# BaptisteHudyma/RGB-D-SLAM

Measured on AMD Instinct MI355X. Metric: depth frames/s primitive extraction (640x480), higher is better.
Workload: dtype f64; 1 GPU; 640x480 synthetic planar-room depth stream, plane extraction only (BASELINE.json configs[1]); stream_frames=4096, unique_frames_per_gpu=4096, scene=room, sub_batches=0, frames_rendered_on=device (torch)

## Files before the change

rgb-d-slam_amd/csrc/cape_cell_acc.h:

```cpp
#pragma once
#include <hip/hip_runtime.h>

#include "cape_device.h"
#include "cape_internal.h"

namespace cape {


#ifndef CAPE_A_GROUP
#define CAPE_A_GROUP 2
#endif
#ifndef CAPE_A_WAVES
#define CAPE_A_WAVES 4
#endif

constexpr int kThreadsA = 320;
constexpr int kBandThreads = 160;
[[maybe_unused]] constexpr int kPartStride = 11;

struct PxAcc
{
    double S[9];
    uint32_t n;
    uint32_t zminBits1, zmaxBits;
};

__device__ __forceinline__ float acc_px(float zr, double a, double b, PxAcc& A)
{
    const bool valid = zr > 0.0f;
    const float z = valid ? zr : 0.0f;
    A.n += valid ? 1u : 0u;
    const double zd = (double)z;
    const float x = (float)(zd * a);
    const float y = (float)(zd * b);
    A.S[0] += (double)x;
    A.S[1] += (double)y;
    A.S[2] += zd;
    A.S[3] += (double)(x * x);
    A.S[4] += (double)(y * y);
    A.S[5] += (double)(z * z);
    A.S[6] += (double)(x * y);
    A.S[7] += (double)(y * z);
    A.S[8] += (double)(x * z);
    return z;
}

__device__ __forceinline__ uint32_t acc_px_fast(float z, double a, double b, PxAcc& A)
{
    const uint32_t bits = __float_as_uint(z);
    A.n += min(bits, 1u);
    const double zd = (double)z;
    const float x = (float)(zd * a);
    const float y = (float)(zd * b);
    A.S[0] += (double)x;
    A.S[1] += (double)y;
    A.S[2] += zd;
    A.S[3] += (double)(x * x);
    A.S[4] += (double)(y * y);
    A.S[5] += (double)(z * z);
    A.S[6] += (double)(x * y);
    A.S[7] += (double)(y * z);
    A.S[8] += (double)(x * z);
    return bits;
}

__device__ __forceinline__ void acc_f4(const float4& v, double a0, double a1, double a2, double a3, double b, PxAcc& A)
{
    const uint32_t bx = acc_px_fast(v.x, a0, b, A);
    const uint32_t by = acc_px_fast(v.y, a1, b, A);
    const uint32_t bz = acc_px_fast(v.z, a2, b, A);
    const uint32_t bw = acc_px_fast(v.w, a3, b, A);
    A.zmaxBits = max(max(A.zmaxBits, bx), max(by, max(bz, bw)));
    A.zminBits1 = min(min(A.zminBits1, bx - 1u), min(by - 1u, min(bz - 1u, bw - 1u)));
}

__device__ __forceinline__ bool is_continuous(float pixelDepth, float& last)
{
    if (pixelDepth > 0)
    {
        if ((double)fabsf(pixelDepth - last) <= 4.0 * depth_quantization((double)pixelDepth))
        {
            last = pixelDepth;
            return true;
        }
        return false;
    }
    return true;
}

__device__ __forceinline__ bool is_continuous_flat(float pixelDepth, float& last)
{
    const bool positive = pixelDepth > 0;
    const bool close = (double)fabsf(pixelDepth - last) <= 4.0 * depth_quantization((double)pixelDepth);
    last = (positive & close) ? pixelDepth : last;
    return !positive | close;
}

}
```

rgb-d-slam_amd/csrc/cape_cell_moments.hip:

```cpp
#include <hip/hip_runtime.h>

#include <type_traits>

#include "cape_cell_acc.h"

namespace cape {

template <bool U16> __global__ __launch_bounds__(kThreadsA, CAPE_A_WAVES) void cape_cell_moments_kernel(StageAParams p)
{
    __shared__ double s_part[kThreadsA * kPartStride];
    __shared__ float s_row[64 * kCell];
    __shared__ float s_col[64 * kCell];
    __shared__ float s_corner[64 * 2];
    __shared__ float s_trash[kThreadsA + kCell];

    const int t = threadIdx.x;
    const int frame = blockIdx.x / p.pairsPerFrame;
    const int pair = blockIdx.x - frame * p.pairsPerFrame;
    const size_t frameOff = (size_t)frame * p.W * p.H;

    const int bsel = t / kBandThreads;
    const int q = t - bsel * kBandThreads;
    const int band = pair * 2 + bsel;
    const int cellRow = band / p.segsPerRow;
    const int seg = band - cellRow * p.segsPerRow;
    const int col0 = seg * 640 + q * 4;
    const bool active = (band < p.bandsPerFrame) && (col0 < p.W);
    const int cseg = q / 5;
    const int j = q - cseg * 5;
    const int lcell = bsel * 32 + cseg;

    PxAcc A;
#pragma unroll
    for (int k = 0; k < 9; ++k)
        A.S[k] = 0.0;
    A.n = 0;
    A.zminBits1 = 0xFFFFFFFFu;
    A.zmaxBits = 0u;
    if (active)
    {
        const double a0 = p.acol[col0], a1 = p.acol[col0 + 1], a2 = p.acol[col0 + 2], a3 = p.acol[col0 + 3];
        const uint32_t pixOff32 = (uint32_t)(cellRow * kCell) * (uint32_t)p.W + (uint32_t)col0;
        const float* frameBase = p.depth + frameOff;
        const uint16_t* frameBase16 = p.depth_u16 + frameOff;
        const float scale16 = p.u16_scale;
        const double* brow = p.brow + cellRow * kCell;
        const size_t W = (size_t)p.W;

        constexpr int kGroup = CAPE_A_GROUP, kGroups = kCell / kGroup;
        static_assert(kCell % kGroup == 0 && kGroups % 2 == 0, "the ping-pong loop consumes two groups per trip");
        using Raw = typename std::conditional<U16, ushort4, float4>::type;
        Raw bufA[kGroup], bufB[kGroup];
        auto load_group = [&](Raw (&buf)[kGroup], int g) {
#pragma unroll
            for (int i = 0; i < kGroup; ++i)
            {
                const size_t rowOff = (size_t)(kGroup * g + i) * W;
                if constexpr (U16)
                {
                    typedef unsigned short u16x4 __attribute__((ext_vector_type(4)));
                    const u16x4 v = __builtin_nontemporal_load(reinterpret_cast<const u16x4*>((frameBase16 + rowOff) + pixOff32));
                    buf[i] = make_ushort4(v.x, v.y, v.z, v.w);
                }
                else
                {
                    typedef float f32x4 __attribute__((ext_vector_type(4)));
                    const f32x4 v = __builtin_nontemporal_load(reinterpret_cast<const f32x4*>((frameBase + rowOff) + pixOff32));
                    buf[i] = make_float4(v.x, v.y, v.z, v.w);
                }
            }
        };
        auto to_f4 = [&](const Raw& rw) {
            if constexpr (U16)
            {
                return make_float4((float)rw.x * scale16, (float)rw.y * scale16, (float)rw.z * scale16, (float)rw.w * scale16);
            }
            else
            {
                return rw;
            }
        };
        float* const colp = (j == 2) ? &s_col[lcell * kCell] : &s_trash[t];
        auto sum_group = [&](const Raw (&rawbuf)[kGroup], int g, auto where) {
            constexpr int kWhere = decltype(where)::value;
            float4 buf[kGroup];
#pragma unroll
            for (int i = 0; i < kGroup; ++i)
                buf[i] = to_f4(rawbuf[i]);
#pragma unroll
            for (int i = 0; i < kGroup; ++i)
            {
                const int r = kGroup * g + i;
                acc_f4(buf[i], a0, a1, a2, a3, brow[r], A);
                colp[r] = buf[i].z;
                if (kWhere == 1 && r == kCell / 2)
                    *reinterpret_cast<float4*>(&s_row[lcell * kCell + 4 * j]) = buf[i];
                if (kWhere == 0 && i == 0 && g == 0 && j == 0)
                    s_corner[lcell * 2] = buf[i].x;
                if (kWhere == 2 && r == kCell - 1 && j == 4)
                    s_corner[lcell * 2 + 1] = buf[i].w;
            }
        };
        using First = std::integral_constant<int, 0>;
        using Loop = std::integral_constant<int, 1>;
        using Last = std::integral_constant<int, 2>;
        static_assert(kGroups >= 6 && (kCell / 2) / kGroup >= 2 && (kCell / 2) / kGroup < kGroups - 2, "row 10 belongs to a trip of the loop");
        load_group(bufA, 0);
        load_group(bufB, 1);
        sum_group(bufA, 0, First{});
        load_group(bufA, 2);
        sum_group(bufB, 1, First{});
#pragma unroll 1
        for (int g = 2; g < kGroups - 2; g += 2)
        {
            load_group(bufB, g + 1);
            sum_group(bufA, g, Loop{});
            load_group(bufA, g + 2);
            sum_group(bufB, g + 1, Loop{});
        }
        load_group(bufB, kGroups - 1);
        sum_group(bufA, kGroups - 2, Last{});
        sum_group(bufB, kGroups - 1, Last{});
    }
    {
        double* dst = s_part + t * kPartStride;
#pragma unroll
        for (int k = 0; k < 9; ++k)
            dst[k] = A.S[k];
        dst[9] = (double)A.n;
        reinterpret_cast<uint2*>(dst + 10)[0] = make_uint2(A.zminBits1, A.zmaxBits);
    }
    __syncthreads();

    if (t >= 256)
    {
        const int l = t - 256;
        size_t base[2];
        int lim[2];
#pragma unroll
        for (int cb = 0; cb < 2; ++cb)
        {
            const int bnd = pair * 2 + cb;
            const int cr = bnd / p.segsPerRow;
            const int sg = bnd - cr * p.segsPerRow;
            base[cb] = (size_t)frame * p.cells + cr * p.hCells + sg * 32;
            lim[cb] = bnd < p.bandsPerFrame ? p.hCells - sg * 32 : 0;
        }
#pragma unroll
        for (int k = 0; k < 10; ++k)
        {
            const int e = l + 64 * k;
            const int cell = e / 10;
            const int m = e - cell * 10;
            const int cb = cell >> 5, cs = cell & 31;
            if (cs < (cb ? lim[1] : lim[0]))
            {
                const double* src = s_part + (cb * kBandThreads + cs * 5) * kPartStride + m;
                double acc = src[0];
                acc += src[kPartStride];
                acc += src[2 * kPartStride];
                acc += src[3 * kPartStride];
                acc += src[4 * kPartStride];
                p.cell_sums[((cb ? base[1] : base[0]) + cs) * kSumStride + m] = acc;
            }
        }
        return;
    }

    const int w = t >> 6, l = t & 63;
    const int c64 = w * 16 + (l & 15);
    const bool vertical = (l & 32) != 0;
    const bool second = (l & 16) != 0;
    bool continuous;
    {
        const float* zs = (vertical ? s_col : s_row) + c64 * kCell;
        const float seed = std_maxf(zs[0], zs[1]);
        float last = seed;
#pragma unroll
        for (int i = 1; i <= 9; ++i)
        {
            const float z = zs[i];
            last = (second && z > 0) ? z : last;
        }
        continuous = second || !(seed <= 0);
        const float* zt = zs + (second ? 10 : 1);
        const int steps = second ? (vertical ? 9 : 10) : 9;
#pragma unroll
        for (int k = 0; k < 10; ++k)
        {
            const bool pass = is_continuous_flat(zt[k], last);
            continuous &= pass | (k >= steps);
        }
        continuous &= __shfl_xor((int)continuous, 16) != 0;
        continuous &= __shfl_xor((int)continuous, 32) != 0;
    }
    const int fb = c64 >> 5, fs = c64 & 31;
    const int fband = pair * 2 + fb;
    if ((l >> 4) != 0 || fband >= p.bandsPerFrame)
        return;
    const int fRow = fband / p.segsPerRow;
    const int fSeg = fband - fRow * p.segsPerRow;
    const int fCol = fSeg * 32 + fs;
    if (fCol >= p.hCells)
        return;
    uint32_t zminBits1 = 0xFFFFFFFFu, zmaxBits = 0u;
    uint32_t n = 0;
    {
        const int pbase = fb * kBandThreads + fs * 5;
#pragma unroll
        for (int k = 0; k < 5; ++k)
        {
            const uint2 zr = reinterpret_cast<const uint2*>(s_part + (pbase + k) * kPartStride + 10)[0];
            zminBits1 = min(zminBits1, zr.x);
            zmaxBits = max(zmaxBits, zr.y);
            n += (uint32_t)s_part[(pbase + k) * kPartStride + 9];
        }
    }
    const float zmin = __uint_as_float(zminBits1 + 1u), zmax = __uint_as_float(zmaxBits);
    const float rab = fmaxf(p.ratio_col[fCol], p.ratio_row[fRow]);
    const bool exact_ok = zmaxBits <= 0x7F7FFFFFu && ((n == 0) || (zmax * rab <= 512.0f * zmin));

    const size_t gcell = (size_t)frame * p.cells + fRow * p.hCells + fCol;
    CellAux aux;
    aux.z0 = s_corner[c64 * 2];
    aux.z399 = s_corner[c64 * 2 + 1];
    aux.flags = (n & kCountMask) | (continuous ? kAuxContinuous : 0u) | (exact_ok ? kAuxExact : 0u);
    aux.zc = s_row[c64 * kCell + kCell / 2];
    p.cell_aux[gcell] = aux;
}

hipError_t launch_cell_moments(const StageAParams& p, int nFrames, hipStream_t stream)
{
    const int grid = nFrames * p.pairsPerFrame;
    if (p.depth)
        hipLaunchKernelGGL(cape_cell_moments_kernel<false>, dim3(grid), dim3(kThreadsA), 0, stream, p);
    else
        hipLaunchKernelGGL(cape_cell_moments_kernel<true>, dim3(grid), dim3(kThreadsA), 0, stream, p);
    return hipGetLastError();
}

}
```

Baseline: 2.325 million frames/s.

## Use f32 continuity test with f64 fallback and hoist band indexing to scalars

Replaces the per-pixel f64 depth-continuity check in the scan waves with an f32 polynomial check. The check flags near-threshold cases, and the wave falls back to the exact f64 path only if any lane is unsure. Band row/segment/offset calculations are computed once per block as wave-uniform scalars via readfirstlane, which removes per-thread integer divisions. The reduce wave is restructured so each element index serves both bands. A profiling script that inventories VALU instructions by kernel region is added. The f32 path risks divergence from the f64 results only inside the guarded margin, and the fallback costs a second pass when triggered.

```diff
diff --git a/profiles/a1_inventory.py b/profiles/a1_inventory.py
--- /dev/null
+++ b/profiles/a1_inventory.py
@@ -0,0 +1,101 @@
+#!/usr/bin/env python3
+import argparse
+import os
+import re
+import subprocess
+import sys
+
+sys.path.insert(0, os.path.dirname(os.path.abspath(__file__)))
+from valu_issue import CSRC, RATE_NS, classify
+
+SYMBOLS = (("f32", "_ZN4cape24cape_cell_moments_kernelILb0EEEvNS_12StageAParamsE"),
+           ("u16", "_ZN4cape24cape_cell_moments_kernelILb1EEEvNS_12StageAParamsE"))
+ORDER = ("prologue", "first trips", "loop trip", "last trips", "partial store", "reduce wave", "scan waves", "scan f64 redo", "aux store")
+WEIGHT = {"prologue": 1, "first trips": 1, "loop trip": 3, "last trips": 1, "partial store": 1, "reduce wave": 0.2, "scan waves": 0.8,
+          "scan f64 redo": 0.0, "aux store": 0.8}
+
+
+def find(body, lo, pred):
+    return next(i for i in range(lo, len(body)) if pred(body[i]))
+
+
+def regions(asm, symbol):
+    start = next(i for i, ln in enumerate(asm) if ln.startswith(symbol + ":"))
+    end = find(asm, start, lambda ln: "s_endpgm" in ln)
+    body = asm[start + 1:end + 1]
+    is_depth_load = lambda ln: re.search(r"global_load_dwordx[24] .* nt$", ln.rstrip()) is not None
+    first_load = find(body, 0, is_depth_load)
+    head = find(body, 0, lambda ln: "Loop Header" in ln)
+    label = body[head].split(":")[0]
+    loop_end = find(body, head, lambda ln: re.search(r"s_c?branch\w*\s+" + re.escape(label) + r"\b", ln) is not None)
+    skip = re.search(r"s_cbranch_execz\s+(\S+)", body[find(body, 0, lambda ln: "s_cbranch_execz" in ln)]).group(1)
+    join = find(body, loop_end, lambda ln: ln.startswith(skip + ":"))
+    barrier = find(body, join, lambda ln: "s_barrier" in ln)
+    out = {"prologue": body[:first_load], "first trips": body[first_load:head], "loop trip": body[head:loop_end + 1],
+           "last trips": body[loop_end + 1:join], "partial store": body[join:barrier + 1]}
+    br = find(body, barrier, lambda ln: re.search(r"s_cbranch_\w+\s+\.LBB", ln) is not None)
+    target = re.search(r"(\.LBB\w+)", body[br]).group(1)
+    split = find(body, br, lambda ln: ln.startswith(target + ":"))
+    arms = [body[barrier + 1:split], body[split:]]
+    reduce_arm = next(a for a in arms if any("global_store_dwordx2" in ln for ln in a))
+    scan_arm = next(a for a in arms if a is not reduce_arm)
+    out["reduce wave"] = reduce_arm
+    last_perm = max(i for i, ln in enumerate(scan_arm) if "ds_bpermute_b32" in ln)
+    scan, redo = scan_arm[:last_perm + 1], []
+    for i, ln in enumerate(scan):
+        m = re.search(r"s_cbranch_vccz\s+(\.LBB\w+)", ln)
+        if m:
+            j = find(scan, i, lambda x: x.startswith(m.group(1) + ":"))
+            if any(re.search(r"v_cmp_\w+_f64", x) for x in scan[i:j]):
+                scan, redo = scan[:i + 1] + scan[j:], scan[i + 1:j]
+                break
+    out["scan waves"], out["scan f64 redo"], out["aux store"] = scan, redo, scan_arm[last_perm + 1:]
+    return out
+
+
+def count(lines):
+    c = {"f64": 0, "double_rate": 0, "other": 0}
+    for ln in lines:
+        m = re.match(r"\s+(v_\w+)", ln)
+        if m:
+            c[classify(m.group(1))] += 1
+    return c
+
+
+def inventory(asm):
+    res = {}
+    for variant, symbol in SYMBOLS:
+        res[variant] = {name: count(lines) for name, lines in regions(asm, symbol).items()}
+    return res
+
+
+def priced(c):
+    return sum(c[k] * RATE_NS[k] for k in RATE_NS)
+
+
+def main():
+    ap = argparse.ArgumentParser()
+    ap.add_argument("--asm", default="")
+    args = ap.parse_args()
+    path = args.asm
+    if not path:
+        path = "/tmp/cape_cell_moments.inventory.s"
+        flags = "-O3 -std=c++17 -fPIC --offload-arch=gfx950 -ffp-contract=off -fno-fast-math -fno-slp-vectorize".split()
+        subprocess.check_call(["/opt/rocm/bin/hipcc"] + flags + ["-S", "--cuda-device-only", "-o", path, os.path.join(CSRC, "cape_cell_moments.hip")],
+                              stderr=subprocess.DEVNULL)
+    inv = inventory(open(path).read().splitlines())
+    for variant, regs in inv.items():
+        print(f"{variant}   VALU instructions as listed                      f64-rate  double-rate  other   total   runs/wave   issue ns/wave")
+        tot_n = tot_ns = 0.0
+        for name in ORDER:
+            c = regs[name]
+            n = c["f64"] + c["double_rate"] + c["other"]
+            ns = priced(c) * WEIGHT[name]
+            tot_n += n * WEIGHT[name]
+            tot_ns += ns
+            print(f"  {name:<48} {c['f64']:8d} {c['double_rate']:12d} {c['other']:6d} {n:7d} {WEIGHT[name]:11.1f} {ns:15.1f}")
+        print(f"  {'per wave, weighted':<48} {'':8} {'':12} {'':6} {tot_n:7.0f} {'':11} {tot_ns:15.1f}")
+
+
+if __name__ == "__main__":
+    main()
diff --git a/rgb-d-slam_amd/csrc/cape_cell_acc.h b/rgb-d-slam_amd/csrc/cape_cell_acc.h
--- a/rgb-d-slam_amd/csrc/cape_cell_acc.h
+++ b/rgb-d-slam_amd/csrc/cape_cell_acc.h
@@ -96,4 +96,19 @@
     return !positive | close;
 }
 
+__device__ __forceinline__ bool is_continuous_flat_f32(float pixelDepth, float& last, bool& unsure)
+{
+    constexpr float c2 = (float)(4.0 * (2.73 * ((1.0 / 1000.0) * (1.0 / 1000.0))));
+    constexpr float c1 = (float)(4.0 * (0.74 / 1000.0));
+    constexpr float c0 = (float)(4.0 * -0.53);
+    const bool positive = pixelDepth > 0;
+    const float r = fmaxf(fmaf(fmaf(c2, pixelDepth, c1), pixelDepth, c0), 2.0f);
+    const float t = fabsf(pixelDepth - last) - r;
+    const bool notSure = !(fabsf(t) > r * 0x1p-16f);
+    const bool close = t <= 0;
+    unsure |= positive & notSure;
+    last = (positive & close) ? pixelDepth : last;
+    return !positive | close;
 }
+
+}
diff --git a/rgb-d-slam_amd/csrc/cape_cell_moments.hip b/rgb-d-slam_amd/csrc/cape_cell_moments.hip
--- a/rgb-d-slam_amd/csrc/cape_cell_moments.hip
+++ b/rgb-d-slam_amd/csrc/cape_cell_moments.hip
@@ -19,13 +19,23 @@
     const int pair = blockIdx.x - frame * p.pairsPerFrame;
     const size_t frameOff = (size_t)frame * p.W * p.H;
 
+    const int band0 = pair * 2;
+    const int cellRow0 = band0 / p.segsPerRow;
+    const int seg0 = band0 - cellRow0 * p.segsPerRow;
+    const bool wrap = seg0 + 1 == p.segsPerRow;
+    const int cellRowOf[2] = {cellRow0, cellRow0 + (wrap ? 1 : 0)};
+    const int segOf[2] = {seg0, wrap ? 0 : seg0 + 1};
+    const bool bandExists[2] = {band0 < p.bandsPerFrame, band0 + 1 < p.bandsPerFrame};
+    const int firstRowOf[2] = {__builtin_amdgcn_readfirstlane(cellRowOf[0] * kCell), __builtin_amdgcn_readfirstlane(cellRowOf[1] * kCell)};
+    const int firstColOf[2] = {__builtin_amdgcn_readfirstlane(segOf[0] * 640), __builtin_amdgcn_readfirstlane(segOf[1] * 640)};
+    const uint32_t firstPixOf[2] = {(uint32_t)__builtin_amdgcn_readfirstlane(firstRowOf[0] * p.W), (uint32_t)__builtin_amdgcn_readfirstlane(firstRowOf[1] * p.W)};
+    const int colLimitOf[2] = {bandExists[0] ? p.W : 0, bandExists[1] ? p.W : 0};
+
     const int bsel = t / kBandThreads;
     const int q = t - bsel * kBandThreads;
-    const int band = pair * 2 + bsel;
-    const int cellRow = band / p.segsPerRow;
-    const int seg = band - cellRow * p.segsPerRow;
-    const int col0 = seg * 640 + q * 4;
-    const bool active = (band < p.bandsPerFrame) && (col0 < p.W);
+    const int row0 = bsel ? firstRowOf[1] : firstRowOf[0];
+    const int col0 = (bsel ? firstColOf[1] : firstColOf[0]) + q * 4;
+    const bool active = col0 < (bsel ? colLimitOf[1] : colLimitOf[0]);
     const int cseg = q / 5;
     const int j = q - cseg * 5;
     const int lcell = bsel * 32 + cseg;
@@ -40,11 +50,11 @@
     if (active)
     {
         const double a0 = p.acol[col0], a1 = p.acol[col0 + 1], a2 = p.acol[col0 + 2], a3 = p.acol[col0 + 3];
-        const uint32_t pixOff32 = (uint32_t)(cellRow * kCell) * (uint32_t)p.W + (uint32_t)col0;
+        const uint32_t pixOff32 = (bsel ? firstPixOf[1] : firstPixOf[0]) + (uint32_t)col0;
         const float* frameBase = p.depth + frameOff;
         const uint16_t* frameBase16 = p.depth_u16 + frameOff;
         const float scale16 = p.u16_scale;
-        const double* brow = p.brow + cellRow * kCell;
+        const double* brow = p.brow + row0;
         const size_t W = (size_t)p.W;
 
         constexpr int kGroup = CAPE_A_GROUP, kGroups = kCell / kGroup;
@@ -132,42 +142,44 @@
     }
     __syncthreads();
 
-    if (t >= 256)
-    {
-        const int l = t - 256;
-        size_t base[2];
+    const int w = __builtin_amdgcn_readfirstlane(t >> 6);
+    if (w == 4)
+    {
+        const int l = t & 63;
+        static_assert(kBandThreads == 32 * 5 && kSumStride == 10, "a band is 32 cells of 5 partials, a cell 10 sums");
+        double* dst[2];
         int lim[2];
 #pragma unroll
         for (int cb = 0; cb < 2; ++cb)
         {
-            const int bnd = pair * 2 + cb;
-            const int cr = bnd / p.segsPerRow;
-            const int sg = bnd - cr * p.segsPerRow;
-            base[cb] = (size_t)frame * p.cells + cr * p.hCells + sg * 32;
-            lim[cb] = bnd < p.bandsPerFrame ? p.hCells - sg * 32 : 0;
-        }
-#pragma unroll
-        for (int k = 0; k < 10; ++k)
-        {
-            const int e = l + 64 * k;
-            const int cell = e / 10;
-            const int m = e - cell * 10;
-            const int cb = cell >> 5, cs = cell & 31;
-            if (cs < (cb ? lim[1] : lim[0]))
-            {
-                const double* src = s_part + (cb * kBandThreads + cs * 5) * kPartStride + m;
-                double acc = src[0];
-                acc += src[kPartStride];
-                acc += src[2 * kPartStride];
-                acc += src[3 * kPartStride];
-                acc += src[4 * kPartStride];
-                p.cell_sums[((cb ? base[1] : base[0]) + cs) * kSumStride + m] = acc;
+            dst[cb] = p.cell_sums + ((size_t)frame * p.cells + cellRowOf[cb] * p.hCells + segOf[cb] * 32) * kSumStride;
+            lim[cb] = bandExists[cb] ? p.hCells - segOf[cb] * 32 : 0;
+        }
+#pragma unroll
+        for (int k = 0; k < 5; ++k)
+        {
+            const int o = l + 64 * k;
+            const int cs = o / kSumStride;
+            const double* src = s_part + o + (5 * kPartStride - kSumStride) * cs;
+#pragma unroll
+            for (int cb = 0; cb < 2; ++cb)
+            {
+                if (cs < lim[cb])
+                {
+                    const double* sp = src + cb * kBandThreads * kPartStride;
+                    double acc = sp[0];
+                    acc += sp[kPartStride];
+                    acc += sp[2 * kPartStride];
+                    acc += sp[3 * kPartStride];
+                    acc += sp[4 * kPartStride];
+                    dst[cb][o] = acc;
+                }
             }
         }
         return;
     }
 
-    const int w = t >> 6, l = t & 63;
+    const int l = t & 63;
     const int c64 = w * 16 + (l & 15);
     const bool vertical = (l & 32) != 0;
     const bool second = (l & 16) != 0;
@@ -175,32 +187,50 @@
     {
         const float* zs = (vertical ? s_col : s_row) + c64 * kCell;
         const float seed = std_maxf(zs[0], zs[1]);
-        float last = seed;
+        float start = seed;
 #pragma unroll
         for (int i = 1; i <= 9; ++i)
         {
             const float z = zs[i];
-            last = (second && z > 0) ? z : last;
-        }
-        continuous = second || !(seed <= 0);
+            start = (second && z > 0) ? z : start;
+        }
+        const bool seeded = second || !(seed <= 0);
         const float* zt = zs + (second ? 10 : 1);
         const int steps = second ? (vertical ? 9 : 10) : 9;
+        float zk[10];
 #pragma unroll
         for (int k = 0; k < 10; ++k)
-        {
-            const bool pass = is_continuous_flat(zt[k], last);
+            zk[k] = zt[k];
+        float last = start;
+        bool unsure = false;
+        continuous = seeded;
+#pragma unroll
+        for (int k = 0; k < 10; ++k)
+        {
+            bool stepUnsure = false;
+            const bool pass = is_continuous_flat_f32(zk[k], last, stepUnsure);
             continuous &= pass | (k >= steps);
+            unsure |= stepUnsure & (k < steps);
+        }
+        if (__any(unsure))
+        {
+            last = start;
+            continuous = seeded;
+#pragma unroll
+            for (int k = 0; k < 10; ++k)
+            {
+                const bool pass = is_continuous_flat(zk[k], last);
+                continuous &= pass | (k >= steps);
+            }
         }
         continuous &= __shfl_xor((int)continuous, 16) != 0;
         continuous &= __shfl_xor((int)continuous, 32) != 0;
     }
-    const int fb = c64 >> 5, fs = c64 & 31;
-    const int fband = pair * 2 + fb;
-    if ((l >> 4) != 0 || fband >= p.bandsPerFrame)
+    const int fb = w >> 1, fs = (w & 1) * 16 + (l & 15);
+    if ((l >> 4) != 0 || !(fb ? bandExists[1] : bandExists[0]))
         return;
-    const int fRow = fband / p.segsPerRow;
-    const int fSeg = fband - fRow * p.segsPerRow;
-    const int fCol = fSeg * 32 + fs;
+    const int fRow = fb ? cellRowOf[1] : cellRowOf[0];
+    const int fCol = (fb ? segOf[1] : segOf[0]) * 32 + fs;
     if (fCol >= p.hCells)
         return;
     uint32_t zminBits1 = 0xFFFFFFFFu, zmaxBits = 0u;
```

Result: faster. 2.359 million frames/s (median of 6 runs) (+1.4%).
